# fukangl/SMG-multimodal-grasping

Hardware: AMD Instinct MI355X
Metric: affordance fwd+bwd passes/sec (16-rot 224^2 RGB-D) (higher is better)
Workload: dtype f32; 1 GPU; 16 rot x 224^2 (S=640): fwd + Huber + bwd + Adam per GPU per step; reinforcement_net style 0; 17 trunk passes; fp32; leg=headline, rotations=16, input_size=640, parallelism=dp1

## Files before the change

### smg-multimodal-grasping_amd/csrc/backward.hip

```cpp
#include "engine.h"

int do_backward(smg_engine* e, const smg_net* net, const float* dq, hipStream_t st, int phases, bool elem_head) {
    if (!e->have_fwd) return fail(-22, "smg_backward without a preceding smg_forward");
    if (!net->grads) return fail(-22, "net.grads is NULL");
    if (phases == 2 && !e->bw_phase0_done)
        return fail(-22, "smg_backward_phase(1) must follow smg_backward_phase(0) of the same forward");
    if ((phases & 1) && e->bw_phase0_done)
        return fail(-22, "smg_backward / smg_backward_phase(0) while the second half of a two-phase backward is still due (run phase 1 or a new forward)");
    const Layout& L = *e->L;
    const TrunkRef& T = L.trunk[e->f_trunk];
    const HeadRef& Hd = L.head[e->f_head];
    const int NS = e->f_streams, NP = e->f_pairs;
    const float* P = net->params;
    float* Gr = net->grads;
    const Plane p4 = e->p_blk[3];
    const bool ph_a = phases & 1, ph_b = phases & 2;
    if (ph_a) {
        for (int r = 0; r < kStatRep; ++r) HIP_OK(hipMemsetAsync(e->bstat + (size_t)r * kStatRepStride, 0, 2 * e->bstat_span * sizeof(double), st));
    }
    const bool split16 = e->prec == 0 && kSplitOp == 3;
    if (ph_a && split16) HIP_OK(hipMemsetAsync(e->gamax, 0, (size_t)e->gamax_words * sizeof(unsigned), st));
    const hipStream_t s2 = (e->prof || e->serialize) ? st : e->side;
    auto fork = [&](hipEvent_t ev) -> int {
        HIP_OK(hipEventRecord(ev, st));
// ... 173 lines not shown
                BwdWeightP<MC<Cfg, decltype(ptag)::value>, W_ONE, C_IDENT, kPdWgrad, false, decltype(ptag)::value> p{};
                p.gbuf = lb.D2; p.ldg = kBottleneck; p.gcoff = 0; p.xbuf = nullptr; p.pa = pl; p.MA = kBottleneck; p.binv = lb.D2S; p.basc = asc_n1(e, b, i);
                p.bbuf = e->X[b]; p.ldb = Ct; p.pb = pl; p.NB = d.cin;
                p.bsum = fsum(e, e->st_X[b]); p.bsq = fsq(e, e->st_X[b]); p.bstride = Ct; p.btab = stat_table(e, e->sx_tab[b], e->max_streams, Ct);
                p.bgamma = P + d.n1.w; p.bbeta = P + d.n1.b; p.eps = kEps;
                p.chunk = w.chunk; p.chunks_per_stream = w.cps; p.n_chunks = NS * w.cps;
                p.dw = Gr + d.c1.w; p.ldw_out = d.cin;
                const dim3 grid(1, w.nt, NS * w.cps);
                return launch_wgrad(e, s2, p, grid, K_W1, 2.0 * NS * pl.HW * d.cin * kBottleneck,
                                    ESZ(e) * NS * pl.HW * (kBottleneck + d.cin), 1, C_IDENT, tiles, tiles.place_behind3x3(wgrad_partial_floats(p, grid)));
            };
            PREC_DISPATCH(e, if (int rc = go(PTAG)) return rc);
        }
        return 0;
    };
    auto debug_stop = [&]() -> int {
        launch_reduce2(e, s2, tiles.drain());
        HIP_OK(hipEventRecord(e->ev_end, s2));
        HIP_OK(hipStreamWaitEvent(st, e->ev_end, 0));
        if (int rc = walk_status(e)) return rc;
        e->have_fwd = false; e->bw_phase0_done = false; e->prof_stage = -1;
        return 0;
    };
    for (int b = ph_a ? 3 : 0; b >= (ph_b ? 0 : 1); --b) {
        e->prof_stage = b;
        const Plane pl = e->p_blk[b];
        const int Ct = kBlockCtot[b];
        if (e->dbg_stop == b * 100 + 50) return debug_stop();
        for (int i = (int)T.layers[b].size() - 1; i >= 0; --i) {
            const DenseLayerRef& d = T.layers[b][i];
            float* bt = el(e, e->Bt, e->bt_off[b][i]);
            const LayerBuf lb = buf_of(b, i);
            float* GSb = lb.GS;
            float* D2b = lb.D2;
            static_assert(kRing % 3 == 0 && kRing > 3, "the sparse ring wait covers three slots at a time");
            if (lb.ring >= kRing && lb.ring % 3 == 0) HIP_OK(hipStreamWaitEvent(st, e->ev_side[(lb.ring + 2) % kRing], 0));
            GradSrc gsrc = fused_gsrc(b, d);
            if (e->generic3x3 || (gs_materialised && !gs_on_side(pl))) {
                launch_gs_apply(b, i, st, GSb);
                if (gs_materialised) { gsrc = GradSrc{}; gsrc.g = GSb; gsrc.ldg = kGrowth; gsrc.amax = gamax_of(e, b, i, 0); }
            }
            if (!e->generic3x3) {
                Halo3x3DgradArgs a;
                a.g = gsrc; a.pl = pl; a.C = kBottleneck;
                a.mbuf = bt;
                a.dst = split16 ? e->DY2 : D2b; a.o1 = b1(e, e->st_Bt[b][i]); a.o2 = b2(e, e->st_Bt[b][i]); a.ostride = kBottleneck;
                a.wu = e->packed_u + e->pk_hd[b][i]; a.bt = bn_table(e, e->sb_tab[b][i], e->max_streams, 0, kBottleneck, P + d.n2.w, P + d.n2.b);
                const double flops = 2.0 * NS * pl.HW * 9 * kBottleneck * kGrowth;
                const double bytes = ESZ(e) * NS * pl.HW * (kGrowth + 2 * kBottleneck);
                if (halo_tile(pl, NS) == 16) {
                    a.tiles_x = (pl.W + 15) / 16; a.cg_per_wg = kBottleneck / 32;
// ... 131 lines not shown
            }
            {
                auto run = [&](auto tag, auto ptag) {
                using Cfg = MC<decltype(tag), decltype(ptag)::value>;
                BwdDataP<Cfg, false, E_UNPOOL, true, decltype(ptag)::value> p{};
                p.gbuf = e->G[b]; p.ldg = Ct; p.gcoff = 0; p.xbuf = e->X[b]; p.ldx = Ct; p.xcoff = 0; p.pa = pl; p.KA = C0;
                p.xsum = fsum(e, e->st_X[b]); p.xsq = fsq(e, e->st_X[b]); p.xstride = Ct;
                p.s1 = b1(e, e->st_X[b]); p.s2 = b2(e, e->st_X[b]); p.sstride = Ct; p.scoff = 0; p.agamma = nullptr;
                p.wp = e->packed_u + e->pk_td[b - 1]; p.K8tot = C0 / 8; p.ldn = Cp; p.wcol0 = 0; p.N = Cp;
                p.mbuf = e->X[b - 1]; p.ldm = Cp; p.mcoff = 0; p.pm = pp;
                p.msum = fsum(e, e->st_X[b - 1]); p.msq = fsq(e, e->st_X[b - 1]); p.mstride = Cp;
                p.egamma = P + T.tnorm[b - 1].w; p.ebeta = P + T.tnorm[b - 1].b;
                p.dst = e->G[b - 1]; p.ldd = Cp; p.dcoff = 0;
                p.o1 = b1(e, e->st_X[b - 1]); p.o2 = b2(e, e->st_X[b - 1]); p.ostride = Cp; p.ocoff = 0;
                p.dbeta = e->dbscr + e->db_toff[b - 1]; p.dgamma = e->dbscr + e->db_toff[b - 1] + Cp; p.rep_stride = e->db_total; p.eps = kEps;
                launch_gemm(e, st, p, dim3(NS * pl.HWp / Cfg::BM, Cp / Cfg::BN), K_TD, 2.0 * NS * pl.HW * Cp * C0,
                            ESZ(e) * NS * (2.0 * pl.HW * C0 + 2.0 * pp.HW * Cp));
            };
            PREC_DISPATCH(e, run(CfgP64x128{}, PTAG));
            }
        }
    }
    e->prof_stage = -1;
    if (ph_b) {
    {
        Pool0BwdArgs a;
        a.G1 = e->G[0]; a.X1 = e->X[0]; a.ld1 = kBlockCtot[0]; a.p1 = e->p_blk[0];
        a.xsum = fsum(e, e->st_X[0]); a.xsq = fsq(e, e->st_X[0]); a.xstride = kBlockCtot[0];
        a.SA = b1(e, e->st_X[0]); a.SB = b2(e, e->st_X[0]); a.sstride = kBlockCtot[0];
        a.argmax = e->argmax; a.stem = e->stem; a.ps = e->p_stem;
        a.ssum = fsum(e, e->st_stem); a.ssq = fsq(e, e->st_stem);
        a.gamma = P + T.norm0.w; a.beta = P + T.norm0.b; a.eps = kEps;
        a.DY0 = e->DY0; a.o1 = b1(e, e->st_stem); a.o2 = b2(e, e->st_stem);
        a.dbeta = Gr + T.norm0.b; a.dgamma = Gr + T.norm0.w;
        if (e->p_stem.H % 8 || e->p_stem.W % 8) return fail(-22, "stem plane must tile by 8 (input_size multiple of 16)");
        a.tiles_per_wg = 8;
        const int n_t = (e->p_stem.H / 8) * (e->p_stem.W / 8);
        PREC_DISPATCH(e, launch_kernel(e, pool0_bwd_kernel<PREC>, dim3((n_t + a.tiles_per_wg - 1) / a.tiles_per_wg, NS), dim3(256), 0, st, K_OTHER, 0, 0, false, a));
    }
    {
        const Plane ps_ = e->p_stem;
        int chunk, cps;
        pick_chunk(ps_, NS, 1, chunk, cps);
        auto go = [&](auto ptag, auto mtag) -> int {
        constexpr int SM = decltype(mtag)::value;
        using WCfg = typename std::conditional<SM == W_STEM1, CfgW64x64, CfgW64x256>::type;
        BwdWeightP<WCfg, SM, SM == W_STEM1 ? C_STEM1 : C_STEM, kPdWgrad, true, decltype(ptag)::value> p{};
// ... 33 lines not shown
```

### smg-multimodal-grasping_amd/csrc/elem.cuh

```cuda
#pragma once
#include "gemm.cuh"

namespace smg {

struct PrepArgs {
    const float* images_nchw;
    const double* heightmaps;
    int hm, pad, S;
    double mean, stdv;
    const int* stream_image;
    const float* stream_affine;
    const int* stream_rotated;
    float* img4;
    float* img1;
    int HWp;
    const double* masks;
    const int* stream_mask_a;
    const int* stream_mask_b;
};

__device__ __forceinline__ float lin_coord(int i, int S, float step) {
    return (i < S / 2) ? fmaf(step, (float)i, -1.f) : fmaf(-step, (float)(S - 1 - i), 1.f);
}

// ... 191 lines not shown
struct BnStatArgs {
    const double* sum; const double* sq; int sstride;
    float eps; double inv_count;
    float* mean; float* invstd; int ld;
    int c0, C, rows;
};
static __global__ void bn_stat_kernel(const BnStatArgs a) {
    const int idx = blockIdx.x * blockDim.x + threadIdx.x;
    if (idx >= a.rows * a.C) return;
    const int n = idx / a.C, c = a.c0 + idx - n * a.C;
    float mean, invstd;
    bn_moments(a.sum, a.sq, (int64_t)n * a.sstride + c, a.inv_count, a.eps, mean, invstd);
    a.mean[(int64_t)n * a.ld + c] = mean;
    a.invstd[(int64_t)n * a.ld + c] = invstd;
}

struct Pool0Args {
    const float* stem; Plane ps;
    const double* ssum; const double* ssq;
    const float* gamma; const float* beta; float eps;
    void* x1; int ldx; Plane po;
    double* dsum; double* dsq; int dstride;
    unsigned char* argmax;
};

template <int PREC>
static __global__ __launch_bounds__(256) void pool0_kernel(const Pool0Args a) {
    using XT = act_t<PREC>;
    __shared__ float prm[192];
    __shared__ double red[2][16][64];
    const int n = blockIdx.y, t = threadIdx.x, cq = t & 15, slot = t >> 4;
    if (t < 64) {
        float mean, invstd;
        bn_moments(a.ssum, a.ssq, (int64_t)n * 64 + t, 1.0 / (double)a.ps.HW, a.eps, mean, invstd);
        prm[t] = mean;
        prm[64 + t] = a.gamma[t] * invstd;
        prm[128 + t] = a.beta[t];
    }
    __syncthreads();
    double s[4] = {0, 0, 0, 0}, ss[4] = {0, 0, 0, 0};
    for (int i = 0; i < 4; ++i) {
        const int p = blockIdx.x * 64 + slot + 16 * i;
        if (p >= a.po.HW) continue;
        const int y = p / a.po.W, x = p - y * a.po.W;
        float best[4] = {-INFINITY, -INFINITY, -INFINITY, -INFINITY};
        int bi[4] = {0, 0, 0, 0};
        for (int k = 0; k < 9; ++k) {
            const int yy = 2 * y - 1 + k / 3, xx = 2 * x - 1 + k % 3;
            if ((unsigned)yy >= (unsigned)a.ps.H || (unsigned)xx >= (unsigned)a.ps.W) continue;
            const float4 v = bnrelu4(ld4(a.stem + ((int64_t)n * a.ps.HWp + yy * a.ps.W + xx) * 64 + 4 * cq), prm + 4 * cq, 64);
            const float vv[4] = {v.x, v.y, v.z, v.w};
#pragma unroll
            for (int c = 0; c < 4; ++c)
                if (vv[c] > best[c]) { best[c] = vv[c]; bi[c] = k; }
        }
        const int64_t o = (int64_t)n * a.po.HWp + p;
        stq<XT>(a.x1, o * a.ldx + 4 * cq, make_float4(best[0], best[1], best[2], best[3]));
        if (a.argmax) *reinterpret_cast<uchar4*>(a.argmax + o * 64 + 4 * cq) = make_uchar4(bi[0], bi[1], bi[2], bi[3]);
#pragma unroll
        for (int c = 0; c < 4; ++c) { s[c] += (double)best[c]; ss[c] += (double)best[c] * (double)best[c]; }
    }
#pragma unroll
    for (int c = 0; c < 4; ++c) { red[0][slot][4 * cq + c] = s[c]; red[1][slot][4 * cq + c] = ss[c]; }
    __syncthreads();
    if (t < 128) {
        const int q = t >> 6, c = t & 63;
        double tot = 0.0;
        for (int k = 0; k < 16; ++k) tot += red[q][k][c];
        atomicAdd((q ? a.dsq : a.dsum) + (int64_t)n * a.dstride + c + fstat_rep(), tot);
    }
}

struct FeatArgs {
    const void* x4; Plane p4;
    const double* xsum; const double* xsq;
    const float* gamma; const float* beta; float eps;
    const int* pair_a; const int* pair_b;
    float* F;
    double* fsum; double* fsq;
    int chunk;
};
// ... 637 lines not shown
#pragma unroll
                for (int c = 0; c < 4; ++c)
                    if (al[pp][4 * cq + c] == k) g[c] += gl[pp][4 * cq + c];
            }
        const float st[4] = {sv[i].x, sv[i].y, sv[i].z, sv[i].w};
        float dy[4];
#pragma unroll
        for (int c = 0; c < 4; ++c) {
            dy[c] = bn1(st[c], prm[128 + 4 * cq + c], prm[4 * cq + c], prm[64 + 4 * cq + c]) > 0.f ? g[c] : 0.f;
            s1[c] += dy[c];
            s2[c] += dy[c] * ((st[c] - prm[128 + 4 * cq + c]) * prm[192 + 4 * cq + c]);
        }
        *reinterpret_cast<float4*>(a.DY0 + srow[i] * 64 + 4 * cq) = make_float4(dy[0], dy[1], dy[2], dy[3]);
    }
    }
#pragma unroll
    for (int c = 0; c < 4; ++c) { red[0][slot][4 * cq + c] = s1[c]; red[1][slot][4 * cq + c] = s2[c]; }
    __syncthreads();
    if (t < 128) {
        const int q = t >> 6, c = t & 63;
        float tot = 0.f;
        for (int k = 0; k < 16; ++k) tot += red[q][k][c];
        atomicAdd((q ? a.o2 : a.o1) + (int64_t)n * 64 + c + stat_rep(), (double)tot);
    }
}

struct BnBwdApplyArgs {
    const void* g; int ldg, gcoff;
    const void* x; int ldx, xcoff;
    Plane pl; int C;
    const double* xsum; const double* xsq; int xstride; StatTab xtab;
    const double* s1; const double* s2; int sstride, scoff;
    const float* gamma; float eps;
    void* out; int ldo;
    float* dbeta; float* dgamma;
    unsigned* amax;
};

constexpr int bn_apply_rows(int prec) { return prec ? 128 : 64; }
template <int PREC>
static __global__ __launch_bounds__(256) void bn_bwd_apply_kernel(const BnBwdApplyArgs a) {
    using XT = act_t<PREC>;
    using GT = grd_t<PREC>;
    constexpr int E = 16 / GT::size;
    constexpr int RPW = bn_apply_rows(PREC);
    static_assert(GT::size == XT::size, "one slot geometry");
// ... 379 lines not shown
```

### smg-multimodal-grasping_amd/csrc/engine.h

```cpp
#pragma once
#include <hip/hip_runtime.h>

#include <algorithm>
#include <cmath>
#include <cstdio>
#include <cstdlib>
#include <cstring>
#include <string>
#include <type_traits>
#include <vector>

#include "../../include/smg_hip.h"
#include "elem.cuh"
#include "scene.cuh"
#include "gemm.cuh"
#include "halo.cuh"
#include "ws.cuh"
#include "wsw.cuh"
#include "plan.h"

using namespace smg;

int smg_fail(int code, const std::string& msg);
static inline int fail(int code, const std::string& msg) { return smg_fail(code, msg); }
// ... 69 lines not shown
    int max_pack = 0;
    float* asc = nullptr; ActScaleDesc* d_asc = nullptr; int n_asc = 0;
    unsigned* gamax = nullptr; int64_t gamax_words = 0;
    float* stab = nullptr; int64_t stab_floats = 0;
    int64_t sx_tab[4] = {}, sb_tab[4][24] = {}, sf_tab = 0;
    BnUpdDesc* d_bnupd = nullptr;
    bool have_fwd = false; int f_trunk = 0, f_head = 0, f_streams = 0, f_pairs = 0;
    bool bw_phase0_done = false;
    bool f_dense_dq = false;
    int head_bwd = 0;
    bool f_stem1 = false;
    int* d_stream_image = nullptr; int* d_stream_rot = nullptr; int* d_pair_a = nullptr; int* d_pair_b = nullptr;
    int* d_seq_t = nullptr; int* d_seq_h = nullptr; int* d_user_ptr = nullptr; int* d_user_pair = nullptr; int* d_user_slot = nullptr;
    float* d_affine = nullptr;
    float* scene_val = nullptr; int* scene_idx = nullptr; int scene_tiles = 0;
    int* d_stage = nullptr; int* h_stage[2] = {}; hipEvent_t ev_stage[2] = {}; int stage_ints = 0, stage_turn = 0;
    int so_image = 0, so_rot = 0, so_pa = 0, so_pb = 0, so_seq_t = 0, so_seq_h = 0, so_uptr = 0, so_upair = 0, so_uslot = 0, so_aff = 0, so_ma = 0, so_mb = 0, so_adam = 0;
    bool capturing = false; int* h_stage_g = nullptr; hipEvent_t ev_graph = nullptr, ev_gin = nullptr; hipStream_t gstream = nullptr; struct StepGraph* step_graph = nullptr;
    int64_t workspace_bytes = 0;
    int n_cu = 256;
    int prec = 0;
    bool serialize = false;
    bool deterministic = false;
    bool generic3x3 = false, generic_c1 = false, generic_w1 = false;
    int dbg_stop = -1;
    float* dbg_gsnap = nullptr; int64_t dbg_gsnap_floats = 0;
    bool prof = false; std::vector<ProfRec> recs; std::vector<hipEvent_t> ev_pool;
    double prof_ms[5][K_COUNT] = {}; int64_t prof_n[5][K_COUNT] = {}; double prof_flops[5][K_COUNT] = {}; double prof_bytes[5][K_COUNT] = {}; int prof_stage = -1;
    int launch_rc = 0;
};

static Plane make_plane(int H, int W) {
    Plane p; p.H = H; p.W = W; p.HW = H * W;
    const int g = p.HW >= 8192 ? 128 : 64;
    p.HWp = (p.HW + g - 1) / g * g;
    return p;
}

template <class T>
static int dev_alloc(smg_engine* e, T** out, int64_t count) {
    void* p = nullptr;
    hipError_t err = hipMalloc(&p, (size_t)count * sizeof(T));
    if (err != hipSuccess) return fail(-12, std::string("hipMalloc ") + std::to_string(count * sizeof(T)) + " B: " + hipGetErrorString(err));
    e->workspace_bytes += count * (int64_t)sizeof(T);
    *out = (T*)p;
    return 0;
}
#define ALLOC(ptr, count) do { int _r = dev_alloc(e, &(ptr), (count)); if (_r) return _r; } while (0)

static hipEvent_t prof_event(smg_engine* e) {
    if (!e->ev_pool.empty()) { hipEvent_t ev = e->ev_pool.back(); e->ev_pool.pop_back(); return ev; }
    hipEvent_t ev; (void)hipEventCreate(&ev); return ev;
}
// ... 184 lines not shown
```

### smg-multimodal-grasping_amd/csrc/engine.hip

```cpp
#include "engine.h"

static thread_local std::string g_err;
int smg_fail(int code, const std::string& msg) { g_err = msg; return code; }

static int engine_build(smg_engine* e) {
    const Layout& L = *e->L;
    const int NS = e->max_streams, NP = e->max_pairs;
    const int S = e->S;
    const int H1 = (S - 1) / 2 + 1, H2 = (H1 - 1) / 2 + 1;
    e->p_img = make_plane(S, S);
    e->p_stem = make_plane(H1, H1);
    int h = H2;
    for (int b = 0; b < 4; ++b) { e->p_blk[b] = make_plane(h, h); h /= 2; }
    e->OH = e->OW = e->p_blk[3].H - kHeadKernel + 1;
    if (e->OH < 1) return fail(-22, "input_size too small for the 20x20 value head");

    if (getenv("SMG_SERIALIZE")) e->serialize = true;
    const int cross = getenv("SMG_CROSSCHECK") ? atoi(getenv("SMG_CROSSCHECK")) : 0;
    e->generic3x3 = cross & 1; e->generic_c1 = cross & 2; e->generic_w1 = cross & 4;

    ALLOC(e->img4, (int64_t)NS * e->p_img.HWp * 4);
    ALLOC(e->stem, (int64_t)NS * e->p_stem.HWp * 64);
    ALLOC(e->DY0, (int64_t)NS * e->p_stem.HWp * 64);
    ALLOC(e->argmax, (int64_t)NS * e->p_blk[0].HWp * 64);
    int64_t bt_total = 0;
    for (int b = 0; b < 4; ++b) {
        ALLOC(e->X[b], (int64_t)NS * e->p_blk[b].HWp * kBlockCtot[b]);
        ALLOC(e->G[b], (int64_t)NS * e->p_blk[b].HWp * kBlockCtot[b]);
        for (int i = 0; i < kBlockLayers[b]; ++i) {
            e->bt_off[b].push_back(bt_total);
            bt_total += (int64_t)NS * e->p_blk[b].HWp * kBottleneck;
        }
    }
    ALLOC(e->Bt, bt_total);
    for (int k = 0; k < kRing; ++k) {
        ALLOC(e->D2[k], (int64_t)NS * e->p_blk[0].HWp * kBottleneck);
        ALLOC(e->GS[k], (int64_t)NS * e->p_blk[0].HWp * kGrowth);
        ALLOC(e->D2S[k], (int64_t)NS * (e->p_blk[0].HWp / kScaleBlock));
        HIP_OK(hipEventCreateWithFlags(&e->ev_gs[k], hipEventDisableTiming));
        HIP_OK(hipEventCreateWithFlags(&e->ev_d2[k], hipEventDisableTiming));
        HIP_OK(hipEventCreateWithFlags(&e->ev_side[k], hipEventDisableTiming));
    }
    ALLOC(e->DY2, (int64_t)NS * e->p_blk[0].HWp * kBottleneck);
    e->scene_tiles = (int)(((int64_t)(S / 2) * (S / 2) + kSceneTile - 1) / kSceneTile);
    ALLOC(e->scene_val, (int64_t)kSceneMaps * e->scene_tiles);
    ALLOC(e->scene_idx, (int64_t)kSceneMaps * e->scene_tiles);
    HIP_OK(hipEventCreateWithFlags(&e->ev_misc, hipEventDisableTiming));
// ... 296 lines not shown
    int ndev = 0;
    if (hipGetDeviceCount(&ndev) != hipSuccess || ndev <= 0) return fail(-19, "no HIP device available: the affordance engine needs an MI355X");
    if (device < 0 || device >= ndev) return fail(-22, "device index out of range");
    HIP_OK(hipSetDevice(device));
    smg_engine* e = new smg_engine();
    e->device = device; e->S = input_size; e->max_streams = max_streams; e->max_pairs = max_pairs; e->head_out = head_out;
    e->L = &layout_for(head_out);
    {
        int cus = 0;
        if (hipDeviceGetAttribute(&cus, hipDeviceAttributeMultiprocessorCount, device) == hipSuccess && cus > 0) e->n_cu = cus;
    }
    int r = engine_build(e);
    if (r) { smg_engine_destroy(e); return r; }
    *out = e;
    return 0;
}

void smg_engine_destroy(smg_engine* e) {
    if (!e) return;
    (void)hipSetDevice(e->device);
    (void)hipDeviceSynchronize();
    void* ptrs[] = {e->img4, e->stem, e->DY0, e->argmax, e->X[0], e->X[1], e->X[2], e->X[3], e->G[0], e->G[1], e->G[2], e->G[3],
                    e->Bt, e->DY2, e->part, e->F, e->DF, e->H1, e->DH1, e->fstat, e->bstat, e->dbscr, e->d_dbseg, e->asc, e->d_asc, e->gamax, e->packed_u, e->packed_f, e->stab, e->d_pack, e->d_bnupd,
                    e->d_stage, e->scene_val, e->scene_idx};
    for (void* p : ptrs) if (p) (void)hipFree(p);
    if (e->dbg_gsnap) (void)hipFree(e->dbg_gsnap);
    step_graph_drop(e);
    if (e->h_stage_g) (void)hipHostFree(e->h_stage_g);
    if (e->ev_graph) (void)hipEventDestroy(e->ev_graph);
    if (e->ev_gin) (void)hipEventDestroy(e->ev_gin);
    if (e->gstream) (void)hipStreamDestroy(e->gstream);
    for (int k = 0; k < 2; ++k) { if (e->h_stage[k]) (void)hipHostFree(e->h_stage[k]); if (e->ev_stage[k]) (void)hipEventDestroy(e->ev_stage[k]); }
    for (int k = 0; k < kRing; ++k) {
        if (e->D2[k]) (void)hipFree(e->D2[k]);
        if (e->GS[k]) (void)hipFree(e->GS[k]);
        if (e->D2S[k]) (void)hipFree(e->D2S[k]);
        if (e->ev_gs[k]) (void)hipEventDestroy(e->ev_gs[k]); if (e->ev_d2[k]) (void)hipEventDestroy(e->ev_d2[k]); if (e->ev_side[k]) (void)hipEventDestroy(e->ev_side[k]);
    }
    if (e->ev_misc) (void)hipEventDestroy(e->ev_misc);
    if (e->ev_end) (void)hipEventDestroy(e->ev_end);
    if (e->side) (void)hipStreamDestroy(e->side);
    for (auto& r : e->recs) { (void)hipEventDestroy(r.a); (void)hipEventDestroy(r.b); }
    for (auto ev : e->ev_pool) (void)hipEventDestroy(ev);
    delete e;
}

int64_t smg_engine_workspace_bytes(const smg_engine* e) { return e ? e->workspace_bytes : 0; }
// ... 525 lines not shown
```

### smg-multimodal-grasping_amd/csrc/forward.hip

```cpp
#include "engine.h"

int validate_batch(const smg_engine* e, const smg_batch* B) {
    const int NS = B->n_streams, NP = B->n_pairs;
    if (NS < 1 || NS > e->max_streams || NP < 1 || NP > e->max_pairs) return fail(-22, "batch exceeds engine capacity");
    if (!B->images_nchw_dev && !B->heightmaps_dev) return fail(-22, "no input images");
    for (int s = 0; s < NS; ++s)
        if (B->stream_image[s] < 0 || B->stream_image[s] >= B->n_images) return fail(-22, "stream_image out of range");
    if (B->masks_dev) {
        if (!B->heightmaps_dev || !B->stream_mask_a || !B->stream_mask_b) return fail(-22, "device masks need the heightmap input form and both index arrays");
        for (int s = 0; s < NS; ++s)
            if (B->stream_mask_a[s] >= B->n_masks || B->stream_mask_b[s] >= B->n_masks || (B->stream_mask_a[s] < 0 && B->stream_mask_b[s] >= 0))
                return fail(-22, "stream mask index out of range");
    }
    for (int j = 0; j < NP; ++j)
        if (B->pair_a[j] < 0 || B->pair_a[j] >= NS || B->pair_b[j] < 0 || B->pair_b[j] >= NS) return fail(-22, "pair index out of range");
    const int n_seq_t = B->bn_seq_trunk ? B->n_bn_seq_trunk : 0, n_seq_h = B->bn_seq_head ? B->n_bn_seq_head : 0;
    const int R = e->max_streams > e->max_pairs ? e->max_streams : e->max_pairs;
    if (n_seq_t > 4 * R + 16 || n_seq_h > 4 * R + 16) return fail(-22, "bn sequence too long");
    if (B->heightmaps_dev) {
        const int pad = (e->S - 2 * B->hm_size) / 2;
        if (pad < 0 || 2 * B->hm_size + 2 * pad != e->S) return fail(-22, "heightmap size does not match engine input_size");
    }
    return 0;
}
// ... 83 lines not shown
        }
        if (head_unit) {
            auto run = [&](auto tag, auto ptag, auto mtag) {
                using Cfg = decltype(tag);
                constexpr int SM = decltype(mtag)::value;
                FwdConvP<Cfg, SM, decltype(ptag)::value> p{};
                p.src = img4; p.lds_ = 4; p.ps = e->p_img; p.po = e->p_stem; p.K = 0;
                p.wp = e->packed_u + (SM == F_STEM1 ? e->pk_conv0_1 : e->pk_conv0); p.K8tot = (SM == F_STEM1 ? 64 : 224) / 8; p.N = 64;
                p.dst = stem; p.ldd = 64; p.dcoff = 0;
                p.dsum = st_off(fsum(e, e->st_stem), 64); p.dsq = st_off(fsq(e, e->st_stem), 64); p.dstride = 64;
                launch_gemm(e, cs, p, dim3(ns * e->p_stem.HWp / Cfg::BM, 1), K_STEM, 2.0 * ns * e->p_stem.HW * 64 * 147,
                            4.0 * ns * ((double)e->p_img.HW * (SM == F_STEM1 ? 1 : 4) + (double)e->p_stem.HW * 64));
            };
            if (stem1) { PREC_DISPATCH(e, if (e->p_stem.HWp % 128 == 0) run(CfgP128x64{}, PTAG, std::integral_constant<int, F_STEM1>{}); else run(CfgP64x64{}, PTAG, std::integral_constant<int, F_STEM1>{})); }
            else { PREC_DISPATCH(e, if (e->p_stem.HWp % 128 == 0) run(CfgP128x64{}, PTAG, std::integral_constant<int, F_STEM>{}); else run(CfgP64x64{}, PTAG, std::integral_constant<int, F_STEM>{})); }
        }
        if (head_unit) {
            Pool0Args a;
            a.stem = stem; a.ps = e->p_stem; a.ssum = st_off(fsum(e, e->st_stem), 64); a.ssq = st_off(fsq(e, e->st_stem), 64);
            a.gamma = P + T.norm0.w; a.beta = P + T.norm0.b; a.eps = kEps;
            a.x1 = xs(0); a.ldx = kBlockCtot[0]; a.po = e->p_blk[0];
            a.dsum = st_off(fsum(e, e->st_X[0]), kBlockCtot[0]); a.dsq = st_off(fsq(e, e->st_X[0]), kBlockCtot[0]); a.dstride = kBlockCtot[0];
            a.argmax = e->argmax + (int64_t)s0 * e->p_blk[0].HWp * 64;
            PREC_DISPATCH(e, launch_kernel(e, pool0_kernel<PREC>, dim3(e->p_blk[0].HWp / 64, ns), dim3(256), 0, cs, K_OTHER, 0, 0, false, a));
        }
        for (int b = 0; b < 4; ++b) {
            e->prof_stage = b;
            const Plane pl = e->p_blk[b];
            const int Ct = kBlockCtot[b];
            double* xsum = st_off(fsum(e, e->st_X[b]), Ct); double* xsq = st_off(fsq(e, e->st_X[b]), Ct);
            for (size_t i = 0; i < T.layers[b].size(); ++i) {
                if (!on()) continue;
                const DenseLayerRef& d = T.layers[b][i];
                float* bt = el(e, e->Bt, e->bt_off[b][i] + (int64_t)s0 * pl.HWp * kBottleneck);
                double* bsum = st_off(fsum(e, e->st_Bt[b][i]), kBottleneck); double* bsq = st_off(fsq(e, e->st_Bt[b][i]), kBottleneck);
                {
                    const BnTab t1 = bn_table(e, e->sx_tab[b], e->max_streams, s0, Ct, P + d.n1.w, P + d.n1.b);
                    if (i == 0) bn_stat(cs, t1, ns, xsum, xsq, Ct, 0, d.cin, pl.HW);
                    auto run_p = [&](auto tag, auto ptag) {
                        using Cfg0 = decltype(tag);
                        using Cfg = MC<Cfg0, decltype(ptag)::value, (Cfg0::BK < 32 ? 2 : 1)>;
                        FwdConvP<Cfg, F_ONE, decltype(ptag)::value> p{};
                        p.src = xs(b); p.lds_ = Ct; p.ps = pl; p.po = pl; p.K = d.cin; p.asc = asc_n1(e, b, (int)i);
                        p.bt = t1; p.fresh0 = i == 0 ? d.cin : d.cin - kGrowth; p.fsum = xsum; p.fsq = xsq; p.fstride = Ct; p.eps = kEps;
                        p.tw_mean = const_cast<float*>(t1.mean); p.tw_invstd = const_cast<float*>(t1.invstd);
                        p.wp = e->packed_u + e->pk_c1[b][i]; p.K8tot = d.cin / 8; p.N = kBottleneck;
// ... 154 lines not shown
```

Measured before the change: 63.55 passes/s.

## Compute stem conv weight gradient at pooled resolution plus image moment correction

```diff
diff --git a/smg-multimodal-grasping_amd/csrc/backward.hip b/smg-multimodal-grasping_amd/csrc/backward.hip
--- a/smg-multimodal-grasping_amd/csrc/backward.hip
+++ b/smg-multimodal-grasping_amd/csrc/backward.hip
@@ -219,11 +219,23 @@
         e->have_fwd = false; e->bw_phase0_done = false; e->prof_stage = -1;
         return 0;
     };
+    const bool pooled_tail = e->prec == 0 && e->f_stem1 && !e->stem_plane_tail && (NS > 4 || e->deterministic);
     for (int b = ph_a ? 3 : 0; b >= (ph_b ? 0 : 1); --b) {
         e->prof_stage = b;
         const Plane pl = e->p_blk[b];
         const int Ct = kBlockCtot[b];
         if (e->dbg_stop == b * 100 + 50) return debug_stop();
+        if (b == 0 && pooled_tail) {
+            StemMomArgs a;
+            a.img = e->img4; a.pi = e->p_img; a.ps = e->p_stem; a.part = e->mom_part;
+            a.tiles_x = stem_mom_tiles_x(e->p_stem); a.n_tiles = stem_mom_tiles(e->p_stem); a.tiles_per_wg = kMomTilesPerWg;
+            if (fork(e->ev_misc)) return -5;
+            e->prof_stage = -1;
+            launch_kernel(e, stem_moments_kernel, dim3(e->mom_groups, NS), dim3(256), 0, s2, K_OTHER, 0, 0, false, a);
+            launch_kernel(e, stem_moments_sum_kernel, dim3((kMomOut + 255) / 256, NS), dim3(256), 0, s2, K_OTHER, 0, 0, false,
+                          (const float*)e->mom_part, e->mom_groups, e->mom);
+            e->prof_stage = b;
+        }
         for (int i = (int)T.layers[b].size() - 1; i >= 0; --i) {
             const DenseLayerRef& d = T.layers[b][i];
             float* bt = el(e, e->Bt, e->bt_off[b][i]);
@@ -401,7 +413,38 @@
         }
     }
     e->prof_stage = -1;
-    if (ph_b) {
+    if (ph_b && pooled_tail) {
+        const Plane p1 = e->p_blk[0];
+        StemTailArgs a;
+        a.G1 = e->G[0]; a.X1 = e->X[0]; a.ld1 = kBlockCtot[0]; a.p1 = p1;
+        a.xsum = fsum(e, e->st_X[0]); a.xsq = fsq(e, e->st_X[0]); a.xstride = kBlockCtot[0];
+        a.SA = b1(e, e->st_X[0]); a.SB = b2(e, e->st_X[0]); a.sstride = kBlockCtot[0];
+        a.argmax = e->argmax; a.stemv = e->stemv;
+        a.ssum = fsum(e, e->st_stem); a.ssq = fsq(e, e->st_stem); a.ps = e->p_stem;
+        a.gamma = P + T.norm0.w; a.eps = kEps;
+        a.img = e->img4; a.pi = e->p_img;
+        a.o1 = b1(e, e->st_stem); a.o2 = b2(e, e->st_stem);
+        a.tiles_x = (p1.W + kTailTW - 1) / kTailTW; a.n_tiles = a.tiles_x * ((p1.H + kTailTH - 1) / kTailTH);
+        a.tiles_per_wg = 8;
+        auto groups = [&]() { return (a.n_tiles + a.tiles_per_wg - 1) / a.tiles_per_wg; };
+        while (a.tiles_per_wg < a.n_tiles && ((int64_t)groups() * NS > 3 * e->n_cu || (int64_t)groups() * NS * 64 * 64 > e->part_floats)) ++a.tiles_per_wg;
+        const int Z = groups() * NS;
+        const PartialTiles::Slot at = tiles.place_alone((int64_t)Z * 64 * 64);
+        launch_reduce2(e, s2, at.first);
+        if (at.off < 0) return fail(-12, "partial-gradient workspace too small");
+        a.part = part_at(e, at);
+        HIP_OK(hipEventRecord(e->ev_end, s2));
+        HIP_OK(hipStreamWaitEvent(st, e->ev_end, 0));
+        launch_kernel(e, stem_tail_kernel, dim3(groups(), NS), dim3(256), 0, st, K_SW, 2.0 * NS * p1.HW * 64 * 49,
+                      4.0 * NS * ((double)p1.HW * (3 * 64 + 16) + (double)e->p_img.HW), false, a);
+        if (fork(e->ev_misc)) return -5;
+        launch_reduce2(e, s2, tiles.launched(at, reduce_chunk_major(a.part, Z, 1, 64, 49, 64, 64, Gr + T.conv0.w, 147, C_STEM1)));
+        StemCombineArgs c;
+        c.mom = e->mom; c.w0 = P + T.conv0.w; c.ssum = a.ssum; c.ssq = a.ssq; c.s1 = a.o1; c.s2 = a.o2;
+        c.gamma = a.gamma; c.eps = kEps; c.HW = e->p_stem.HW; c.ns = NS; c.dw = Gr + T.conv0.w;
+        launch_kernel(e, stem_combine_kernel, dim3(64), dim3(256), (size_t)(NS * kMomRows + 256) * sizeof(double), s2, K_OTHER, 0, 0, false, c);
+    }
+    if (ph_b && !pooled_tail) {
     {
         Pool0BwdArgs a;
         a.G1 = e->G[0]; a.X1 = e->X[0]; a.ld1 = kBlockCtot[0]; a.p1 = e->p_blk[0];
diff --git a/smg-multimodal-grasping_amd/csrc/elem.cuh b/smg-multimodal-grasping_amd/csrc/elem.cuh
--- a/smg-multimodal-grasping_amd/csrc/elem.cuh
+++ b/smg-multimodal-grasping_amd/csrc/elem.cuh
@@ -237,6 +237,7 @@
     void* x1; int ldx; Plane po;
     double* dsum; double* dsq; int dstride;
     unsigned char* argmax;
+    float* stemv;
 };
 
 template <int PREC>
@@ -260,18 +261,21 @@
         const int y = p / a.po.W, x = p - y * a.po.W;
         float best[4] = {-INFINITY, -INFINITY, -INFINITY, -INFINITY};
         int bi[4] = {0, 0, 0, 0};
+        float raw[4] = {0.f, 0.f, 0.f, 0.f};
         for (int k = 0; k < 9; ++k) {
             const int yy = 2 * y - 1 + k / 3, xx = 2 * x - 1 + k % 3;
             if ((unsigned)yy >= (unsigned)a.ps.H || (unsigned)xx >= (unsigned)a.ps.W) continue;
-            const float4 v = bnrelu4(ld4(a.stem + ((int64_t)n * a.ps.HWp + yy * a.ps.W + xx) * 64 + 4 * cq), prm + 4 * cq, 64);
-            const float vv[4] = {v.x, v.y, v.z, v.w};
+            const float4 r = ld4(a.stem + ((int64_t)n * a.ps.HWp + yy * a.ps.W + xx) * 64 + 4 * cq);
+            const float4 v = bnrelu4(r, prm + 4 * cq, 64);
+            const float vv[4] = {v.x, v.y, v.z, v.w}, rr[4] = {r.x, r.y, r.z, r.w};
 #pragma unroll
             for (int c = 0; c < 4; ++c)
-                if (vv[c] > best[c]) { best[c] = vv[c]; bi[c] = k; }
+                if (vv[c] > best[c]) { best[c] = vv[c]; bi[c] = k; raw[c] = rr[c]; }
         }
         const int64_t o = (int64_t)n * a.po.HWp + p;
         stq<XT>(a.x1, o * a.ldx + 4 * cq, make_float4(best[0], best[1], best[2], best[3]));
         if (a.argmax) *reinterpret_cast<uchar4*>(a.argmax + o * 64 + 4 * cq) = make_uchar4(bi[0], bi[1], bi[2], bi[3]);
+        if (a.stemv) *reinterpret_cast<float4*>(a.stemv + o * 64 + 4 * cq) = make_float4(raw[0], raw[1], raw[2], raw[3]);
 #pragma unroll
         for (int c = 0; c < 4; ++c) { s[c] += (double)best[c]; ss[c] += (double)best[c] * (double)best[c]; }
     }
@@ -955,6 +959,297 @@
         float tot = 0.f;
         for (int k = 0; k < 16; ++k) tot += red[q][k][c];
         atomicAdd((q ? a.o2 : a.o1) + (int64_t)n * 64 + c + stat_rep(), (double)tot);
+    }
+}
+
+constexpr int kTailTW = 16, kTailTH = 4, kTailIW = 4 * kTailTW + 7, kTailIH = 4 * kTailTH + 7, kTailPitch = 75, kTailGl = 65;
+struct StemTailArgs {
+    const float* G1; const float* X1; int ld1; Plane p1;
+    const double* xsum; const double* xsq; int xstride;
+    const double* SA; const double* SB; int sstride;
+    const unsigned char* argmax; const float* stemv;
+    const double* ssum; const double* ssq; Plane ps;
+    const float* gamma; float eps;
+    const float* img; Plane pi;
+    double* o1; double* o2;
+    float* part;
+    int tiles_x, n_tiles, tiles_per_wg;
+};
+
+template <int T0, int NT>
+__device__ __forceinline__ void stem_tail_taps(float (&acc)[13], const float* gl, const unsigned short* ol, const float* it, int c) {
+#pragma unroll 2
+    for (int q = 0; q < kTailTW * kTailTH; ++q) {
+        const float g = gl[q * kTailGl + c];
+        const float* ip = it + ol[q * 64 + c];
+#pragma unroll
+        for (int j = 0; j < NT; ++j) acc[j] = fmaf(g, ip[((T0 + j) / 7) * kTailPitch + (T0 + j) % 7], acc[j]);
+    }
+}
+template <int T0, int NT>
+__device__ __forceinline__ void stem_tail_put(const float (&acc)[13], float* gl, int c, float a) {
+#pragma unroll
+    for (int j = 0; j < NT; ++j) gl[c * kTailGl + T0 + j] = acc[j] * a;
+}
+
+static __global__ __launch_bounds__(256) void stem_tail_kernel(const StemTailArgs a) {
+    __shared__ float prm[7 * 64];
+    __shared__ float gl[64 * kTailGl];
+    __shared__ unsigned short ol[64 * 64];
+    __shared__ float it[kTailIH * kTailPitch];
+    static_assert(2 * 16 * 64 <= 64 * kTailGl, "the s1 / s2 reduction reuses gl");
+    const int n = blockIdx.y, t = threadIdx.x, cq = t & 15, slot = t >> 4;
+    if (t < 64) {
+        float mean, invstd;
+        bn_moments(a.ssum, a.ssq, (int64_t)n * 64 + t, 1.0 / (double)a.ps.HW, a.eps, mean, invstd);
+        prm[256 + t] = mean; prm[320 + t] = invstd; prm[384 + t] = a.gamma[t] * invstd;
+        const double inv = 1.0 / (double)a.p1.HW;
+        float m1, i1;
+        bn_moments(a.xsum, a.xsq, (int64_t)n * a.xstride + t, inv, a.eps, m1, i1);
+        const float q1 = (float)(stat_get(a.SA, (int64_t)n * a.sstride + t) * inv);
+        const float q2 = (float)(stat_get(a.SB, (int64_t)n * a.sstride + t) * inv);
+        prm[t] = i1; prm[64 + t] = q1; prm[128 + t] = m1; prm[192 + t] = i1 * q2;
+    }
+    float s1[4] = {0, 0, 0, 0}, s2[4] = {0, 0, 0, 0};
+    float acc[13] = {0, 0, 0, 0, 0, 0, 0, 0, 0, 0, 0, 0, 0};
+    const float* img = a.img + (int64_t)n * a.pi.HWp;
+    const int tile0 = blockIdx.x * a.tiles_per_wg, tile1 = min(tile0 + a.tiles_per_wg, a.n_tiles);
+    for (int tile = tile0; tile < tile1; ++tile) {
+        const int ty = tile / a.tiles_x, tx = tile - ty * a.tiles_x;
+        const int qy0 = ty * kTailTH, qx0 = tx * kTailTW;
+        float4 gq[4], xq[4], sq[4];
+        uchar4 aq[4];
+        bool okq[4];
+#pragma unroll
+        for (int i = 0; i < 4; ++i) {
+            const int lp = slot + 16 * i;
+            const int qy = qy0 + (lp >> 4), qx = qx0 + (lp & 15);
+            okq[i] = qy < a.p1.H && qx < a.p1.W;
+            const int64_t pr = (int64_t)n * a.p1.HWp + (okq[i] ? qy * a.p1.W + qx : 0);
+            gq[i] = ld4(a.G1 + pr * a.ld1 + 4 * cq);
+            xq[i] = ld4(a.X1 + pr * a.ld1 + 4 * cq);
+            sq[i] = ld4(a.stemv + pr * 64 + 4 * cq);
+            aq[i] = *reinterpret_cast<const uchar4*>(a.argmax + pr * 64 + 4 * cq);
+        }
+        constexpr int kImg = kTailIH * kTailIW, kImgLoads = (kImg + 255) / 256;
+        float iv[kImgLoads];
+        const int iy0 = 4 * qy0 - 5, ix0 = 4 * qx0 - 5;
+#pragma unroll
+        for (int j = 0; j < kImgLoads; ++j) {
+            const int idx = t + 256 * j, r = idx / kTailIW, cc = idx - r * kTailIW;
+            const int y = iy0 + r, x = ix0 + cc;
+            const bool in = idx < kImg && (unsigned)y < (unsigned)a.pi.H && (unsigned)x < (unsigned)a.pi.W;
+            iv[j] = img[in ? y * a.pi.W + x : 0];
+            if (!in) iv[j] = 0.f;
+        }
+        __syncthreads();
+#pragma unroll
+        for (int j = 0; j < kImgLoads; ++j) {
+            const int idx = t + 256 * j, r = idx / kTailIW, cc = idx - r * kTailIW;
+            if (idx < kImg) it[r * kTailPitch + cc] = iv[j];
+        }
+#pragma unroll
+        for (int i = 0; i < 4; ++i) {
+            const int lp = slot + 16 * i;
+            const float4 gv = affine2(gq[i], xq[i], prm + 4 * cq, 64);
+            const float g4[4] = {gv.x, gv.y, gv.z, gv.w}, x4[4] = {xq[i].x, xq[i].y, xq[i].z, xq[i].w}, v4[4] = {sq[i].x, sq[i].y, sq[i].z, sq[i].w};
+            const int k4[4] = {aq[i].x, aq[i].y, aq[i].z, aq[i].w};
+#pragma unroll
+            for (int c = 0; c < 4; ++c) {
+                const bool on = okq[i] && x4[c] > 0.f;
+                const float gm = on ? g4[c] : 0.f;
+                s1[c] += gm;
+                s2[c] += gm * ((v4[c] - prm[256 + 4 * cq + c]) * prm[320 + 4 * cq + c]);
+                const int k = on ? k4[c] : 0;
+                gl[lp * kTailGl + 4 * cq + c] = gm;
+                ol[lp * 64 + 4 * cq + c] = (unsigned short)((4 * (lp >> 4) + 2 * (k / 3)) * kTailPitch + 4 * (lp & 15) + 2 * (k % 3));
+            }
+        }
+        __syncthreads();
+        switch (t >> 6) {
+            case 0: stem_tail_taps<0, 13>(acc, gl, ol, it, t & 63); break;
+            case 1: stem_tail_taps<13, 12>(acc, gl, ol, it, t & 63); break;
+            case 2: stem_tail_taps<25, 12>(acc, gl, ol, it, t & 63); break;
+            default: stem_tail_taps<37, 12>(acc, gl, ol, it, t & 63); break;
+        }
+    }
+    __syncthreads();
+    {
+        const int c = t & 63;
+        const float an = prm[384 + c];
+        switch (t >> 6) {
+            case 0: stem_tail_put<0, 13>(acc, gl, c, an); break;
+            case 1: stem_tail_put<13, 12>(acc, gl, c, an); break;
+            case 2: stem_tail_put<25, 12>(acc, gl, c, an); break;
+            default: stem_tail_put<37, 12>(acc, gl, c, an); break;
+        }
+    }
+    __syncthreads();
+    float* po = a.part + ((int64_t)n * gridDim.x + blockIdx.x) * (64 * 64);
+#pragma unroll
+    for (int i = 0; i < 16; ++i) {
+        const int e = t + 256 * i, c = e >> 6, col = e & 63;
+        po[e] = col < 49 ? gl[c * kTailGl + col] : 0.f;
+    }
+    __syncthreads();
+    float* red = gl;
+#pragma unroll
+    for (int c = 0; c < 4; ++c) { red[(0 * 16 + slot) * 64 + 4 * cq + c] = s1[c]; red[(1 * 16 + slot) * 64 + 4 * cq + c] = s2[c]; }
+    __syncthreads();
+    if (t < 128) {
+        const int q = t >> 6, c = t & 63;
+        float tot = 0.f;
+        for (int k = 0; k < 16; ++k) tot += red[(q * 16 + k) * 64 + c];
+        atomicAdd((q ? a.o2 : a.o1) + (int64_t)n * 64 + c + stat_rep(), (double)tot);
+    }
+}
+
+constexpr int kMomT = 16, kMomI = 2 * kMomT + 5, kMomPitch = 39, kMomJobs = 35, kMomSlices = 7, kMomVals = kMomJobs * 49;
+struct StemMomArgs {
+    const float* img; Plane pi; Plane ps;
+    float* part;
+    int tiles_x, n_tiles, tiles_per_wg;
+};
+__host__ __device__ __forceinline__ int stem_mom_block(int ra, int rb) { return ra * 7 - ra * (ra - 1) / 2 + (rb - ra); }
+
+static __global__ __launch_bounds__(256) void stem_moments_kernel(const StemMomArgs a) {
+    __shared__ float it[kMomI * kMomPitch + 8];
+    __shared__ float red[kMomVals];
+    const int n = blockIdx.y, t = threadIdx.x;
+    const int slice = t / kMomJobs, job = t - slice * kMomJobs;
+    int ra = 0, rb = 7;
+    if (job >= 28) ra = job - 28;
+    else {
+        int j = job;
+        while (j >= 7 - ra) { j -= 7 - ra; ++ra; }
+        rb = ra + j;
+    }
+    float acc[7][7];
+#pragma unroll
+    for (int i = 0; i < 7; ++i)
+#pragma unroll
+        for (int j = 0; j < 7; ++j) acc[i][j] = 0.f;
+    if (t < 8) it[kMomI * kMomPitch + t] = t == 0 ? 1.f : 0.f;
+    const float* img = a.img + (int64_t)n * a.pi.HWp;
+    const int tile0 = blockIdx.x * a.tiles_per_wg, tile1 = min(tile0 + a.tiles_per_wg, a.n_tiles);
+    for (int tile = tile0; tile < tile1; ++tile) {
+        const int ty = tile / a.tiles_x, tx = tile - ty * a.tiles_x;
+        const int y0 = ty * kMomT, x0 = tx * kMomT;
+        constexpr int kImg = kMomI * kMomI, kImgLoads = (kImg + 255) / 256;
+        float iv[kImgLoads];
+#pragma unroll
+        for (int j = 0; j < kImgLoads; ++j) {
+            const int idx = t + 256 * j, r = idx / kMomI, cc = idx - r * kMomI;
+            const int y = 2 * y0 - 3 + r, x = 2 * x0 - 3 + cc;
+            const bool in = idx < kImg && (unsigned)y < (unsigned)a.pi.H && (unsigned)x < (unsigned)a.pi.W;
+            iv[j] = img[in ? y * a.pi.W + x : 0];
+            if (!in) iv[j] = 0.f;
+        }
+        __syncthreads();
+#pragma unroll
+        for (int j = 0; j < kImgLoads; ++j) {
+            const int idx = t + 256 * j, r = idx / kMomI, cc = idx - r * kMomI;
+            if (idx < kImg) it[r * kMomPitch + cc] = iv[j];
+        }
+        __syncthreads();
+        if (slice < kMomSlices) {
+            for (int p = slice; p < kMomT * kMomT; p += kMomSlices) {
+                const int ly = p >> 4, lx = p & 15;
+                if (y0 + ly >= a.ps.H || x0 + lx >= a.ps.W) continue;
+                const float* pa = it + (2 * ly + ra) * kMomPitch + 2 * lx;
+                const float* pb = rb < 7 ? it + (2 * ly + rb) * kMomPitch + 2 * lx : it + kMomI * kMomPitch;
+                float av[7], bv[7];
+#pragma unroll
+                for (int i = 0; i < 7; ++i) { av[i] = pa[i]; bv[i] = pb[i]; }
+#pragma unroll
+                for (int i = 0; i < 7; ++i)
+#pragma unroll
+                    for (int j = 0; j < 7; ++j) acc[i][j] = fmaf(av[i], bv[j], acc[i][j]);
+            }
+        }
+    }
+    float tot[7] = {0, 0, 0, 0, 0, 0, 0};
+    for (int s = 0; s < kMomSlices; ++s) {
+        __syncthreads();
+        if (slice == s) {
+#pragma unroll
+            for (int i = 0; i < 7; ++i)
+#pragma unroll
+                for (int j = 0; j < 7; ++j) red[job * 49 + i * 7 + j] = acc[i][j];
+        }
+        __syncthreads();
+#pragma unroll
+        for (int i = 0; i < 7; ++i) {
+            const int e = t + 256 * i;
+            if (e < kMomVals) tot[i] += red[e];
+        }
+    }
+    float* po = a.part + ((int64_t)n * gridDim.x + blockIdx.x) * kMomVals;
+#pragma unroll
+    for (int i = 0; i < 7; ++i) {
+        const int e = t + 256 * i;
+        if (e < kMomVals) po[e] = tot[i];
+    }
+}
+
+constexpr int kMomRows = 50, kMomOut = kMomRows * 49;
+static __global__ void stem_moments_sum_kernel(const float* part, int groups, double* mom) {
+    const int n = blockIdx.y, o = blockIdx.x * blockDim.x + threadIdx.x;
+    if (o >= kMomOut) return;
+    const int u = o / 49, t = o - u * 49, uy = u / 7, ux = u - uy * 7, ty = t / 7, tx = t - ty * 7;
+    const int e = u == 49 ? (28 + ty) * 49 + tx * 7
+                          : uy <= ty ? stem_mom_block(uy, ty) * 49 + ux * 7 + tx : stem_mom_block(ty, uy) * 49 + tx * 7 + ux;
+    double s = 0.0;
+    for (int g = 0; g < groups; ++g) s += (double)part[((int64_t)n * groups + g) * kMomVals + e];
+    mom[(int64_t)n * kMomOut + o] = s;
+}
+
+struct StemCombineArgs {
+    const double* mom; const float* w0;
+    const double* ssum; const double* ssq; const double* s1; const double* s2;
+    const float* gamma; float eps; int HW; int ns;
+    float* dw;
+};
+static __global__ __launch_bounds__(256) void stem_combine_kernel(const StemCombineArgs a) {
+    extern __shared__ double cmb[];
+    double* coef = cmb;
+    double* red = cmb + a.ns * kMomRows;
+    const int c = blockIdx.x, tid = threadIdx.x;
+    const double inv = 1.0 / (double)a.HW;
+    for (int n = tid; n < a.ns; n += 256) {
+        float mean, invstd;
+        bn_moments(a.ssum, a.ssq, (int64_t)n * 64 + c, inv, a.eps, mean, invstd);
+        const float q1 = (float)(stat_get(a.s1, (int64_t)n * 64 + c) * inv);
+        const float q2 = (float)(stat_get(a.s2, (int64_t)n * 64 + c) * inv);
+        const float an = a.gamma[c] * invstd, kk = invstd * q2;
+        coef[n * kMomRows + 48] = -(double)an * (double)kk;
+        coef[n * kMomRows + 49] = (double)an * ((double)kk * (double)mean - (double)q1);
+    }
+    __syncthreads();
+    for (int k = tid; k < a.ns * 49; k += 256) {
+        const int n = k / 49, u = k - n * 49;
+        if (u == 48) continue;
+        coef[n * kMomRows + u] = coef[n * kMomRows + 48] * ((double)a.w0[c * 147 + u] + (double)a.w0[c * 147 + 49 + u] + (double)a.w0[c * 147 + 98 + u]);
+    }
+    __syncthreads();
+    for (int n = tid; n < a.ns; n += 256) coef[n * kMomRows + 48] *= (double)a.w0[c * 147 + 48] + (double)a.w0[c * 147 + 97] + (double)a.w0[c * 147 + 146];
+    __syncthreads();
+    const int t = tid & 63, qt = tid >> 6, K = a.ns * kMomRows;
+    const int k0 = (int)((int64_t)K * qt / 4), k1 = (int)((int64_t)K * (qt + 1) / 4);
+    double v0 = 0.0, v1 = 0.0;
+    if (t < 49) {
+        int k = k0;
+        for (; k + 1 < k1; k += 2) {
+            v0 += coef[k] * a.mom[(int64_t)k * 49 + t];
+            v1 += coef[k + 1] * a.mom[(int64_t)(k + 1) * 49 + t];
+        }
+        if (k < k1) v0 += coef[k] * a.mom[(int64_t)k * 49 + t];
+    }
+    red[qt * 64 + t] = v0 + v1;
+    __syncthreads();
+    if (tid < 49) {
+        const float v = (float)((red[tid] + red[64 + tid]) + (red[128 + tid] + red[192 + tid]));
+        for (int cc = 0; cc < 3; ++cc) a.dw[c * 147 + cc * 49 + tid] += v;
     }
 }
 
diff --git a/smg-multimodal-grasping_amd/csrc/engine.h b/smg-multimodal-grasping_amd/csrc/engine.h
--- a/smg-multimodal-grasping_amd/csrc/engine.h
+++ b/smg-multimodal-grasping_amd/csrc/engine.h
@@ -115,13 +115,19 @@
     int prec = 0;
     bool serialize = false;
     bool deterministic = false;
-    bool generic3x3 = false, generic_c1 = false, generic_w1 = false;
+    bool generic3x3 = false, generic_c1 = false, generic_w1 = false, stem_plane_tail = false;
+    float* stemv = nullptr; float* mom_part = nullptr; double* mom = nullptr; int mom_groups = 0;
     int dbg_stop = -1;
     float* dbg_gsnap = nullptr; int64_t dbg_gsnap_floats = 0;
     bool prof = false; std::vector<ProfRec> recs; std::vector<hipEvent_t> ev_pool;
     double prof_ms[5][K_COUNT] = {}; int64_t prof_n[5][K_COUNT] = {}; double prof_flops[5][K_COUNT] = {}; double prof_bytes[5][K_COUNT] = {}; int prof_stage = -1;
     int launch_rc = 0;
 };
+
+constexpr int kMomTilesPerWg = 8;
+static inline int stem_mom_tiles_x(const Plane& ps) { return (ps.W + kMomT - 1) / kMomT; }
+static inline int stem_mom_tiles(const Plane& ps) { return stem_mom_tiles_x(ps) * ((ps.H + kMomT - 1) / kMomT); }
+static inline int stem_mom_groups(const Plane& ps) { return (stem_mom_tiles(ps) + kMomTilesPerWg - 1) / kMomTilesPerWg; }
 
 static Plane make_plane(int H, int W) {
     Plane p; p.H = H; p.W = W; p.HW = H * W;
diff --git a/smg-multimodal-grasping_amd/csrc/engine.hip b/smg-multimodal-grasping_amd/csrc/engine.hip
--- a/smg-multimodal-grasping_amd/csrc/engine.hip
+++ b/smg-multimodal-grasping_amd/csrc/engine.hip
@@ -17,12 +17,16 @@
 
     if (getenv("SMG_SERIALIZE")) e->serialize = true;
     const int cross = getenv("SMG_CROSSCHECK") ? atoi(getenv("SMG_CROSSCHECK")) : 0;
-    e->generic3x3 = cross & 1; e->generic_c1 = cross & 2; e->generic_w1 = cross & 4;
+    e->generic3x3 = cross & 1; e->generic_c1 = cross & 2; e->generic_w1 = cross & 4; e->stem_plane_tail = cross & 8;
 
     ALLOC(e->img4, (int64_t)NS * e->p_img.HWp * 4);
     ALLOC(e->stem, (int64_t)NS * e->p_stem.HWp * 64);
     ALLOC(e->DY0, (int64_t)NS * e->p_stem.HWp * 64);
     ALLOC(e->argmax, (int64_t)NS * e->p_blk[0].HWp * 64);
+    e->stemv = e->DY0;
+    e->mom_groups = stem_mom_groups(e->p_stem);
+    ALLOC(e->mom_part, (int64_t)NS * e->mom_groups * kMomVals);
+    ALLOC(e->mom, (int64_t)NS * kMomOut);
     int64_t bt_total = 0;
     for (int b = 0; b < 4; ++b) {
         ALLOC(e->X[b], (int64_t)NS * e->p_blk[b].HWp * kBlockCtot[b]);
@@ -365,7 +369,7 @@
     (void)hipDeviceSynchronize();
     void* ptrs[] = {e->img4, e->stem, e->DY0, e->argmax, e->X[0], e->X[1], e->X[2], e->X[3], e->G[0], e->G[1], e->G[2], e->G[3],
                     e->Bt, e->DY2, e->part, e->F, e->DF, e->H1, e->DH1, e->fstat, e->bstat, e->dbscr, e->d_dbseg, e->asc, e->d_asc, e->gamax, e->packed_u, e->packed_f, e->stab, e->d_pack, e->d_bnupd,
-                    e->d_stage, e->scene_val, e->scene_idx};
+                    e->d_stage, e->scene_val, e->scene_idx, e->mom_part, e->mom};
     for (void* p : ptrs) if (p) (void)hipFree(p);
     if (e->dbg_gsnap) (void)hipFree(e->dbg_gsnap);
     step_graph_drop(e);
diff --git a/smg-multimodal-grasping_amd/csrc/forward.hip b/smg-multimodal-grasping_amd/csrc/forward.hip
--- a/smg-multimodal-grasping_amd/csrc/forward.hip
+++ b/smg-multimodal-grasping_amd/csrc/forward.hip
@@ -129,6 +129,7 @@
             a.x1 = xs(0); a.ldx = kBlockCtot[0]; a.po = e->p_blk[0];
             a.dsum = st_off(fsum(e, e->st_X[0]), kBlockCtot[0]); a.dsq = st_off(fsq(e, e->st_X[0]), kBlockCtot[0]); a.dstride = kBlockCtot[0];
             a.argmax = e->argmax + (int64_t)s0 * e->p_blk[0].HWp * 64;
+            a.stemv = (stem1 && e->prec == 0 && !e->stem_plane_tail) ? e->stemv + (int64_t)s0 * e->p_blk[0].HWp * 64 : nullptr;
             PREC_DISPATCH(e, launch_kernel(e, pool0_kernel<PREC>, dim3(e->p_blk[0].HWp / 64, ns), dim3(256), 0, cs, K_OTHER, 0, 0, false, a));
         }
         for (int b = 0; b < 4; ++b) {
```

Measured after the change: 64.19 passes/s, median of 6. 1.0% higher.
